# iostanin1/SCTL

Hardware: AMD Instinct MI355X
Metric: pair-interactions/s, Laplace-SL N x N direct sum (higher is better)
Workload: dtype f64; 1 GPU; Laplace3D single layer (Laplace3D-FxU), 2^20 x 2^20, fp64 [BASELINE headline / north_star target]; kernel=Laplace3D-FxU, n_trg=1048576, n_src=1048576, digits=-1

## Files before the change

include/sctl_amd/device/ukernels.hpp:

```cpp
#pragma once
#include <hip/hip_runtime.h>
#include <stdint.h>
#include <type_traits>

#include "fastmath.hpp"

namespace sctl_amd {

constexpr double kPi = 3.141592653589793238462643383279502884;

struct KerCtx { double v[4]; };

constexpr double kCubicC = 0x1.aaaaaa8000000p+0, kCubicK = 0x1.1c71c6e38e38ep+1;
constexpr double kCubic3C = 0x1.6666660000000p+0, kCubic3K = 0x1.7e4b170a3d700p-2, kCubic5C = 0x1.4924920000000p+0, kCubic5K = 0x1.2cee3c14e5e00p-3;
template <class R> struct RsqConst {
  R c38, c53, k209, c3, k3, c5, k5;
  __device__ __forceinline__ RsqConst() : c38(R(0.375)), c53(R(kCubicC)), k209(R(kCubicK)), c3(R(kCubic3C)), k3(R(kCubic3K)), c5(R(kCubic5C)), k5(R(kCubic5K)) {
    asm volatile("" : "+v"(c38), "+s"(c53), "+s"(k209), "+s"(c3), "+s"(k3), "+s"(c5), "+s"(k5));
  }
};

template <int MODE, bool MASKED> __device__ __forceinline__ double rsqrt_masked(double r2, const RsqConst<double>& K) {
  double y = __builtin_amdgcn_rsq(r2);
  if (MASKED) {
  int hi = __double2hiint(y);
  asm("" : "+v"(hi));
  hi = (hi == 0x7ff00000) ? 0 : hi;
  y = __hiloint2double(hi, __double2loint(y));
  }
  if (MODE >= 1) {
    const double a = r2 * y;
    const double e = __builtin_fma(-a, y, 1.0);
    const double ye = y * e;
    if (MODE == 1) y = __builtin_fma(ye, 0.5, y);
    else y = __builtin_fma(ye, __builtin_fma(e, K.c38, 0.5), y);
  }
  return y;
}
template <int MODE, bool MASKED> __device__ __forceinline__ float rsqrt_masked(float r2, const RsqConst<float>&) {
  float y = __builtin_amdgcn_rsqf(r2);
  if (MASKED) y = (__float_as_uint(y) == 0x7f800000u) ? 0.0f : y;
  if (MODE >= 1) {
    const float a = r2 * y;
    const float e = __builtin_fmaf(-a, y, 1.0f);
    y = __builtin_fmaf(y * e, 0.5f, y);
  }
  return y;
}

template <class R> struct DefaultConsts {
  static constexpr int LDS_DOUBLES = 0;
  static constexpr bool HAS_VARIANT = false;
  RsqConst<R> rsq;
  __device__ __forceinline__ explicit DefaultConsts(double*) {}
  __device__ __forceinline__ void begin_tile() const {}
  __device__ __forceinline__ bool tile_bad(const KerCtx&) const { return false; }
};
constexpr double helmholtz_dist_factor(int mode) { return mode == 1 ? 2.0 : mode == 2 ? 0x1.5555550000000p+1 : 1.0; }
template <class R> struct HelmholtzConsts;
template <> struct HelmholtzConsts<float> {
  static constexpr int LDS_DOUBLES = 0;
  static constexpr bool HAS_VARIANT = true;
  static constexpr int NUM_VARIANTS = 2;
  __device__ __forceinline__ int variant(const KerCtx& ctx) const { return ctx.v[1] == 0 ? 1 : 0; }
  RsqConst<float> rsq;
  float cinv = 1.0f;
  __device__ __forceinline__ explicit HelmholtzConsts(double*) {}
  __device__ __forceinline__ HelmholtzConsts(double*, int, const KerCtx&, int mode) : cinv((float)(1.0 / helmholtz_dist_factor(mode))) {}
  __device__ __forceinline__ void begin_tile() const {}
  __device__ __forceinline__ bool tile_bad(const KerCtx&) const { return false; }
};
template <> struct HelmholtzConsts<double> {
  static constexpr int LDS_DOUBLES = fastmath::kTableDoubles;
  static constexpr int LDS_DOUBLES_ALL_PAIRS = fastmath::kCexpTableDoubles > fastmath::kTableDoubles ? fastmath::kCexpTableDoubles : fastmath::kTableDoubles;
  static constexpr bool HAS_VARIANT = true;
  static constexpr int NUM_VARIANTS = 4;
  bool one_reduction;
  __device__ __forceinline__ int variant(const KerCtx& ctx) const { return (ctx.v[1] == 0 ? 1 : 0) + (one_reduction ? 2 : 0); }
  RsqConst<double> rsq;
  fastmath::TabCoeffsK tk;
  fastmath::CexpCoeffsK ck;
  const double* table;
  double cdist, cinv;
  __device__ __forceinline__ HelmholtzConsts(double* lds, int lds_doubles, const KerCtx& ctx) : HelmholtzConsts(lds, lds_doubles, ctx, 0) {}
  __device__ __forceinline__ HelmholtzConsts(double* lds, int lds_doubles, const KerCtx& ctx, int mode) : table(lds), cdist(helmholtz_dist_factor(mode)), cinv(1.0 / helmholtz_dist_factor(mode)) {
    one_reduction = lds_doubles >= fastmath::kCexpTableDoubles && fastmath::CexpCoeffsK::usable(ctx.v[0], -ctx.v[1]);
    {
      const fastmath::Coeffs full;
      if (one_reduction) fastmath::fill_cexp_tables(lds, (int)threadIdx.x, (int)blockDim.x, ctx.v[0], -ctx.v[1], full, fastmath::TabCoeffs());
      else fastmath::fill_tables(lds, (int)threadIdx.x, (int)blockDim.x, full);
    }
    __syncthreads();
    if (one_reduction) {
      ck.set_scaled(ctx.v[0], -ctx.v[1], fastmath::TabCoeffs(), cdist);
      ck.pin();
    } else {
      tk.set_scaled(ctx.v[0], -ctx.v[1], fastmath::TabCoeffs(), cdist);
      tk.pin();
    }
  }
  __device__ __forceinline__ HelmholtzConsts(double* lds, const KerCtx& ctx) : HelmholtzConsts(lds, LDS_DOUBLES, ctx) {}
  mutable unsigned rmax_hi = 0;
  __device__ __forceinline__ void begin_tile() const { rmax_hi = 0; }
  __device__ __forceinline__ void note_distance(double r) const {
    const unsigned h = (unsigned)__double2hiint(r);
    rmax_hi = (h > rmax_hi) ? h : rmax_hi;
  }
  __device__ __forceinline__ bool tile_bad(const KerCtx& ctx) const {
    const double rmax = __hiloint2double((int)(rmax_hi + 1u), 0);
    if (one_reduction) return !(ctx.v[0] * rmax <= fastmath::kCexpMaxPhase * cdist);
    return !(__builtin_fabs(ctx.v[0]) * rmax <= fastmath::kSincosTabMaxArg * cdist && __builtin_fabs(ctx.v[1]) * rmax <= fastmath::kExpTabMaxArg * cdist);
  }
};

template <class Ker, class R, int MODE, class = void, class = void> struct FinishOf {
  static __device__ __forceinline__ void apply(R (&)[Ker::K1]) {}
};
template <class Ker, class R, int MODE, class V> struct FinishOf<Ker, R, MODE, std::void_t<decltype(&Ker::template finish<R>)>, V> {
  static __device__ __forceinline__ void apply(R (&acc)[Ker::K1]) { Ker::template finish<R>(acc); }
};
template <class Ker, class R, int MODE> struct FinishOf<Ker, R, MODE, void, std::void_t<decltype(&Ker::template finish_mode<R, MODE>)>> {
  static __device__ __forceinline__ void apply(R (&acc)[Ker::K1]) { Ker::template finish_mode<R, MODE>(acc); }
};
template <class Ker, class R, int MODE> __device__ __forceinline__ void finish_acc(R (&acc)[Ker::K1]) { FinishOf<Ker, R, MODE>::apply(acc); }

template <class Ker, class R, int MODE, class = void> struct PackOf {
  static __device__ __forceinline__ void apply(R* rec, const R* x, const R* n, const R* f) { Ker::template pack<R>(rec, x, n, f); }
};
template <class Ker, class R, int MODE> struct PackOf<Ker, R, MODE, std::void_t<decltype(&Ker::template pack_mode<R, MODE>)>> {
  static __device__ __forceinline__ void apply(R* rec, const R* x, const R* n, const R* f) { Ker::template pack_mode<R, MODE>(rec, x, n, f); }
};
template <class Ker, class R, int MODE> __device__ __forceinline__ void pack_record(R* rec, const R* x, const R* n, const R* f) { PackOf<Ker, R, MODE>::apply(rec, x, n, f); }

template <class KC> __device__ __forceinline__ KC make_consts(double* lds, int lds_doubles, const KerCtx& ctx) {
  if constexpr (std::is_constructible<KC, double*, int, const KerCtx&>::value) return KC(lds, lds_doubles, ctx);
  else if constexpr (std::is_constructible<KC, double*, const KerCtx&>::value) return KC(lds, ctx);
  else return KC(lds);
}
template <class KC> __device__ __forceinline__ KC make_consts(double* lds, const KerCtx& ctx) { return make_consts<KC>(lds, KC::LDS_DOUBLES, ctx); }
template <class KC> __device__ __forceinline__ KC make_consts(double* lds, int lds_doubles, const KerCtx& ctx, int mode) {
  if constexpr (std::is_constructible<KC, double*, int, const KerCtx&, int>::value) return KC(lds, lds_doubles, ctx, mode);
  else return make_consts<KC>(lds, lds_doubles, ctx);
}
template <class KC> __device__ __forceinline__ KC make_consts(double* lds, const KerCtx& ctx, int mode) { return make_consts<KC>(lds, KC::LDS_DOUBLES, ctx, mode); }
template <class KC, class = void> struct AllPairsScratch { static constexpr int value = KC::LDS_DOUBLES; };
template <class KC> struct AllPairsScratch<KC, std::void_t<decltype(KC::LDS_DOUBLES_ALL_PAIRS)>> { static constexpr int value = KC::LDS_DOUBLES_ALL_PAIRS; };
template <class KC, class = void> struct NumVariants { static constexpr int value = KC::HAS_VARIANT ? 2 : 1; };
template <class KC> struct NumVariants<KC, std::void_t<decltype(KC::NUM_VARIANTS)>> { static constexpr int value = KC::NUM_VARIANTS; };

template <class R> __device__ __forceinline__ R fma_(R a, R b, R c);
template <> __device__ __forceinline__ double fma_<double>(double a, double b, double c) { return __builtin_fma(a, b, c); }
template <> __device__ __forceinline__ float fma_<float>(float a, float b, float c) { return __builtin_fmaf(a, b, c); }

template <class R> __device__ __forceinline__ R len2(const R (&d)[3]) { return fma_(d[2], d[2], fma_(d[1], d[1], d[0] * d[0])); }
template <class R> __device__ __forceinline__ R dot3(const R (&d)[3], const R* v) { return fma_(d[2], v[2], fma_(d[1], v[1], d[0] * v[0])); }

constexpr double kNewton2MeanErr = -1.725e-16;
constexpr double newton2_factor(int p) { return (p == 1 ? 2.0 : p == 3 ? 8.0 : 32.0) * (1.0 + p * kNewton2MeanErr); }
template <bool MASKED, class R> __device__ __forceinline__ R rsqrt_newton2(R r2, const RsqConst<R>& K) {
  const R y = rsqrt_masked<0, MASKED>(r2, K);
  const R a = r2 * y;
  return y * fma_(-a, y, R(3));
}

constexpr double cubic83_factor(int p) { return p == 1 ? 0x1.5555550000000p+1 : p == 3 ? 0x1.2f684af684bdep+4 : 0x1.0db20937d5dcdp+7; }
template <bool MASKED> __device__ __forceinline__ double rsqrt_cubic83(double r2, const RsqConst<double>& K) {
  const double y = rsqrt_masked<0, MASKED>(r2, K);
  const double z = __builtin_fma(r2, y * y, -K.c53);
  return y * __builtin_fma(z, z, K.k209);
}
template <bool MASKED> __device__ __forceinline__ float rsqrt_cubic83(float r2, const RsqConst<float>& K) { return rsqrt_masked<1, MASKED>(r2, K) * (float)cubic83_factor(1); }
template <int MODE, bool MASKED, class R> __device__ __forceinline__ R rsqrt_scaled(R r2, const RsqConst<R>& K) {
  if constexpr (MODE == 1) return rsqrt_newton2<MASKED>(r2, K);
  else if constexpr (MODE == 2) return rsqrt_cubic83<MASKED>(r2, K);
  else return rsqrt_masked<0, MASKED>(r2, K);
}
constexpr double rsqrt_scaled_factor(int mode, int p) { return mode == 1 ? newton2_factor(p) : mode == 2 ? cubic83_factor(p) : 1; }
constexpr double kCubic3A = 0x1.1111100000000p-1, kCubic5A = 0x1.d41d400000000p-3;
template <bool MASKED> __device__ __forceinline__ double rsqrt3_cubic(double r2, const RsqConst<double>& K) {
  const double y = rsqrt_masked<0, MASKED>(r2, K), s = y * y;
  const double z = __builtin_fma(r2, s, -K.c3);
  return (y * s) * __builtin_fma(z, z, K.k3);
}
template <bool MASKED> __device__ __forceinline__ double rsqrt5_cubic(double r2, const RsqConst<double>& K) {
  const double y = rsqrt_masked<0, MASKED>(r2, K), s = y * y;
  const double z = __builtin_fma(r2, s, -K.c5);
  return (y * (s * s)) * __builtin_fma(z, z, K.k5);
}
constexpr double rsqrt_pow_factor(int mode, int p) { return mode == 2 ? (p == 1 ? cubic83_factor(1) : p == 3 ? kCubic3A : kCubic5A) : rsqrt_scaled_factor(mode, p); }
template <int MODE, int P, bool MASKED, class R> __device__ __forceinline__ R rsqrt_pow_scaled(R r2, const RsqConst<R>& K) {
  static_assert(P == 3 || P == 5, "powers 3 and 5");
  if constexpr (MODE == 2 && std::is_same<R, double>::value) return P == 3 ? rsqrt3_cubic<MASKED>(r2, K) : rsqrt5_cubic<MASKED>(r2, K);
  else if constexpr (MODE == 2) {
    const R y = rsqrt_masked<1, MASKED>(r2, K), y2 = y * y;
    return (P == 3 ? y2 * y : y2 * y2 * y) * R(rsqrt_pow_factor(2, P));
  } else {
    const R y = rsqrt_scaled<MODE, MASKED>(r2, K), y2 = y * y;
    return P == 3 ? y2 * y : y2 * y2 * y;
  }
}

constexpr double rsqrt_scaled_c2(int mode) { return rsqrt_scaled_factor(mode, 1) == 1 ? 1.0 : mode == 1 ? 4.0 : cubic83_factor(1) * cubic83_factor(1); }


constexpr int nrec_multi(int nd, int k0, int m) { return (3 + nd + m * k0 + 1) / 2 * 2; }
template <int ND, int K0, class R, int M> __device__ __forceinline__ void pack_multi(R* rec, const R* x, const R* n, const R (&f)[M][K0]) {
  rec[0] = x[0]; rec[1] = x[1]; rec[2] = x[2];
#pragma unroll
  for (int k = 0; k < ND; k++) rec[3 + k] = n[k];
#pragma unroll
  for (int m = 0; m < M; m++)
#pragma unroll
    for (int k = 0; k < K0; k++) rec[3 + ND + m * K0 + k] = f[m][k];
}
#define SCTL_AMD_MULTI_RECORD                                                                                                          \
  template <int M> static constexpr int NREC_M = nrec_multi(ND, K0, M);                                                               \
  template <class R, int M> static __device__ __forceinline__ void pack_m(R* rec, const R* x, const R* n, const R (&f)[M][K0]) {      \
    pack_multi<ND, K0>(rec, x, n, f);                                                                                                 \
  }

struct Laplace3D_FxU {
  static constexpr int ID = 0, K0 = 1, K1 = 1, ND = 0, NREC = 4, FLOPS = 6;
  static constexpr const char* NAME = "Laplace3D-FxU";
  template <class R> using Consts = DefaultConsts<R>;
  static constexpr double scale() { return 1 / (4 * kPi); }
  static constexpr double acc_factor(int mode) { return rsqrt_scaled_factor(mode, 1); }
  template <class R> static __device__ __forceinline__ void pack(R* rec, const R* x, const R*, const R* f) {
    rec[0] = x[0]; rec[1] = x[1]; rec[2] = x[2]; rec[3] = f[0];
  }
  template <class R, int MODE, bool MASKED> static __device__ __forceinline__ void pair(R (&acc)[K1], const R (&d)[3], const R* rec, const KerCtx&, const Consts<R>& K) {
    const R rinv = rsqrt_scaled<MODE, MASKED>(len2(d), K.rsq);
    acc[0] = fma_(rec[3], rinv, acc[0]);
  }
  SCTL_AMD_MULTI_RECORD
  template <class R, int MODE, bool MASKED, int M> static __device__ __forceinline__ void pair_m(R (&acc)[M][K1], const R (&d)[3], const R* rec, const KerCtx&, const Consts<R>& K) {
    const R rinv = rsqrt_scaled<MODE, MASKED>(len2(d), K.rsq);
#pragma unroll
    for (int m = 0; m < M; m++) acc[m][0] = fma_(rec[3 + m], rinv, acc[m][0]);
  }
};

struct Laplace3D_DxU {
  static constexpr int ID = 1, K0 = 1, K1 = 1, ND = 3, NREC = 6, FLOPS = 14;
  static constexpr const char* NAME = "Laplace3D-DxU";
  template <class R> using Consts = DefaultConsts<R>;
  static constexpr double scale() { return 1 / (4 * kPi); }
  static constexpr double acc_factor(int mode) { return rsqrt_pow_factor(mode, 3); }
  template <class R> static __device__ __forceinline__ void pack(R* rec, const R* x, const R* n, const R* f) {
    rec[0] = x[0]; rec[1] = x[1]; rec[2] = x[2]; rec[3] = n[0] * f[0]; rec[4] = n[1] * f[0]; rec[5] = n[2] * f[0];
  }
  template <class R, int MODE, bool MASKED> static __device__ __forceinline__ void pair(R (&acc)[K1], const R (&d)[3], const R* rec, const KerCtx&, const Consts<R>& K) {
    acc[0] = fma_(dot3(d, rec + 3), rsqrt_pow_scaled<MODE, 3, MASKED>(len2(d), K.rsq), acc[0]);
  }
  SCTL_AMD_MULTI_RECORD
  template <class R, int MODE, bool MASKED, int M> static __device__ __forceinline__ void pair_m(R (&acc)[M][K1], const R (&d)[3], const R* rec, const KerCtx&, const Consts<R>& K) {
    const R t = dot3(d, rec + 3) * rsqrt_pow_scaled<MODE, 3, MASKED>(len2(d), K.rsq);
#pragma unroll
    for (int m = 0; m < M; m++) acc[m][0] = fma_(rec[6 + m], t, acc[m][0]);
  }
};

struct Laplace3D_FxdU {
  static constexpr int ID = 2, K0 = 1, K1 = 3, ND = 0, NREC = 4, FLOPS = 11;
  static constexpr const char* NAME = "Laplace3D-FxdU";
  template <class R> using Consts = DefaultConsts<R>;
  static constexpr double scale() { return -1 / (4 * kPi); }
  static constexpr double acc_factor(int mode) { return rsqrt_pow_factor(mode, 3); }
  template <class R> static __device__ __forceinline__ void pack(R* rec, const R* x, const R*, const R* f) {
    rec[0] = x[0]; rec[1] = x[1]; rec[2] = x[2]; rec[3] = f[0];
  }
  template <class R, int MODE, bool MASKED> static __device__ __forceinline__ void pair(R (&acc)[K1], const R (&d)[3], const R* rec, const KerCtx&, const Consts<R>& K) {
    const R t = rsqrt_pow_scaled<MODE, 3, MASKED>(len2(d), K.rsq) * rec[3];
    for (int j = 0; j < 3; j++) acc[j] = fma_(t, d[j], acc[j]);
  }
  SCTL_AMD_MULTI_RECORD
  template <class R, int MODE, bool MASKED, int M> static __device__ __forceinline__ void pair_m(R (&acc)[M][K1], const R (&d)[3], const R* rec, const KerCtx&, const Consts<R>& K) {
    const R t = rsqrt_pow_scaled<MODE, 3, MASKED>(len2(d), K.rsq);
    const R td[3] = {t * d[0], t * d[1], t * d[2]};
#pragma unroll
    for (int m = 0; m < M; m++)
#pragma unroll
      for (int j = 0; j < 3; j++) acc[m][j] = fma_(rec[3 + m], td[j], acc[m][j]);
  }
};

struct Stokes3D_FxU {
  static constexpr int ID = 3, K0 = 3, K1 = 3, ND = 0, NREC = 10, FLOPS = 23;
  static constexpr const char* NAME = "Stokes3D-FxU";
  template <class R> using Consts = DefaultConsts<R>;
  static constexpr double scale() { return 1 / (8 * kPi); }
  static constexpr double acc_factor(int mode) { return rsqrt_scaled_factor(mode, 3); }
  template <class R, int MODE> static __device__ __forceinline__ void pack_mode(R* rec, const R* x, const R*, const R* f) {
    const R c2 = R(rsqrt_scaled_c2(MODE));
    rec[0] = x[0]; rec[1] = x[1]; rec[2] = x[2]; rec[3] = f[0]; rec[4] = f[1]; rec[5] = f[2]; rec[6] = c2 * f[0]; rec[7] = c2 * f[1]; rec[8] = c2 * f[2]; rec[9] = 0;
  }
  template <class R> static __device__ __forceinline__ void pack(R* rec, const R* x, const R* n, const R* f) { pack_mode<R, 0>(rec, x, n, f); }
  template <class R, int MODE, bool MASKED> static __device__ __forceinline__ void pair(R (&acc)[K1], const R (&d)[3], const R* rec, const KerCtx&, const Consts<R>& K) {
    const R y = rsqrt_scaled<MODE, MASKED>(len2(d), K.rsq);
    const R t = dot3(d, rec + 3) * (y * y);
    for (int j = 0; j < 3; j++) acc[j] = fma_(y, fma_(t, d[j], rec[6 + j]), acc[j]);
  }
  SCTL_AMD_MULTI_RECORD
  template <class R, int MODE, bool MASKED, int M> static __device__ __forceinline__ void pair_m(R (&acc)[M][K1], const R (&d)[3], const R* rec, const KerCtx&, const Consts<R>& K) {
    const R y = rsqrt_scaled<MODE, MASKED>(len2(d), K.rsq);
    const R y3 = (y * y) * y;
    const R yc = (rsqrt_scaled_c2(MODE) == 1.0) ? y : y * R(rsqrt_scaled_c2(MODE));
    const R e[3] = {y3 * d[0], y3 * d[1], y3 * d[2]};
#pragma unroll
    for (int m = 0; m < M; m++) {
      const R* f = rec + 3 + 3 * m;
      const R rf = dot3(d, f);
#pragma unroll
      for (int j = 0; j < 3; j++) acc[m][j] = fma_(e[j], rf, fma_(yc, f[j], acc[m][j]));
    }
  }
};

struct Stokes3D_DxU {
  static constexpr int ID = 4, K0 = 3, K1 = 3, ND = 3, NREC = 10, FLOPS = 26;
  static constexpr const char* NAME = "Stokes3D-DxU";
  template <class R> using Consts = DefaultConsts<R>;
  static constexpr double scale() { return 3 / (4 * kPi); }
  static constexpr double acc_factor(int mode) { return rsqrt_pow_factor(mode, 5); }
  template <class R> static __device__ __forceinline__ void pack(R* rec, const R* x, const R* n, const R* f) {
    for (int k = 0; k < 3; k++) { rec[k] = x[k]; rec[3 + k] = n[k]; rec[6 + k] = f[k]; }
    rec[9] = 0;
  }
  template <class R, int MODE, bool MASKED> static __device__ __forceinline__ void pair(R (&acc)[K1], const R (&d)[3], const R* rec, const KerCtx&, const Consts<R>& K) {
// ... 284 lines not shown
```

sctl_amd/csrc/centered_kernel.hpp:

```cpp
#pragma once
#include <sctl_amd/device/eval_kernel.hpp>

namespace sctl_amd {

constexpr double kNearFactor2 = 4.0;

template <class R> __device__ __forceinline__ R wave_min(R v) {
  for (int o = 32; o > 0; o >>= 1) { const R w = __shfl_xor(v, o); v = (w < v) ? w : v; }
  return v;
}
template <class R> __device__ __forceinline__ R wave_max(R v) {
  for (int o = 32; o > 0; o >>= 1) { const R w = __shfl_xor(v, o); v = (w > v) ? w : v; }
  return v;
}

__device__ __forceinline__ double uniform_(double v) {
  return __hiloint2double(__builtin_amdgcn_readfirstlane(__double2hiint(v)), __builtin_amdgcn_readfirstlane(__double2loint(v)));
}
__device__ __forceinline__ float uniform_(float v) { return __int_as_float(__builtin_amdgcn_readfirstlane(__float_as_int(v))); }
__device__ __forceinline__ double sqrt_(double v) { return __builtin_sqrt(v); }
__device__ __forceinline__ float sqrt_(float v) { return __builtin_sqrtf(v); }

template <class R> struct Rec4;
template <> struct Rec4<double> {
  typedef double V __attribute__((ext_vector_type(2)));
  static constexpr int NW = 2;
  static __device__ __forceinline__ void put(V* p, double a, double b, double c, double d) { p[0] = V{a, b}; p[1] = V{c, d}; }
  static __device__ __forceinline__ void get(const V* p, double (&o)[4]) { const V u = p[0], w = p[1]; o[0] = u[0]; o[1] = u[1]; o[2] = w[0]; o[3] = w[1]; }
};
template <> struct Rec4<float> {
  typedef float V __attribute__((ext_vector_type(4)));
  static constexpr int NW = 1;
  static __device__ __forceinline__ void put(V* p, float a, float b, float c, float d) { p[0] = V{a, b, c, d}; }
  static __device__ __forceinline__ void get(const V* p, float (&o)[4]) { const V u = p[0]; o[0] = u[0]; o[1] = u[1]; o[2] = u[2]; o[3] = u[3]; }
};

constexpr int kWaveBlock = 64;
constexpr int kWaveTile = 64;
#if defined(SCTL_AMD_EXPERIMENTS) && defined(SCTL_AMD_EXP_NEARCAP)
constexpr int kNearCap = SCTL_AMD_EXP_NEARCAP;
static_assert(kNearCap >= 64, "a tile of 64 sources must fit the list of pending near sources");
#else
constexpr int kNearCap = 128;
#endif

typedef float f32x2 __attribute__((ext_vector_type(2)));
template <int MODE, int P = 1> __device__ __forceinline__ f32x2 rsqrt_pair(f32x2 r2) {
  f32x2 y = {__builtin_amdgcn_rsqf(r2[0]), __builtin_amdgcn_rsqf(r2[1])};
  if (MODE >= 1) {
    const f32x2 a = r2 * y;
    y = y * (f32x2{3.0f, 3.0f} - a * y);
    if (MODE == 2) {
      const float k = (float)__builtin_pow(rsqrt_pow_factor(2, P), 1.0 / P) / 2;
      y = y * f32x2{k, k};
    }
  }
  return y;
}
__device__ __forceinline__ f32x2 pk_add_hi(f32x2 t, f32x2 zA) {
  f32x2 r;
  asm("v_pk_add_f32 %0, %1, %2 op_sel:[0,1] op_sel_hi:[1,1]" : "=v"(r) : "v"(t), "v"(zA));
  return r;
}
__device__ __forceinline__ f32x2 pk_fma_lo_hi(f32x2 m, f32x2 g) {
  f32x2 r;
  asm("v_pk_fma_f32 %0, %1, %2, %2 op_sel:[0,0,1] op_sel_hi:[1,0,1]" : "=v"(r) : "v"(m), "v"(g));
  return r;
}

template <class R, int T> struct FarTargets {
  R m2x[T][3], tt[T];
  __device__ __forceinline__ void set(int j, const R (&p)[3], R t2) {
    tt[j] = t2;
#pragma unroll
    for (int k = 0; k < 3; k++) m2x[j][k] = R(-2) * p[k];
  }
};
template <> struct FarTargets<float, 2> {
  f32x2 mp[3], tp;
  __device__ __forceinline__ void set(int j, const float (&p)[3], float t2) {
    tp[j] = t2;
#pragma unroll
    for (int k = 0; k < 3; k++) mp[k][j] = -2.0f * p[k];
  }
};

template <class R> struct CenteredFxU {
  using Ker = Laplace3D_FxU;
  static constexpr bool DUP = std::is_same<R, float>::value;
  static constexpr int XW = DUP ? 2 : 1, NF = 1, NEAR_CAP = 128;
  template <class RR> static constexpr int targets_per_lane() { return sizeof(RR) == 8 ? 4 : 2; }
  struct Extra { R f, f2; };
  template <int MODE> static __device__ __forceinline__ void put_extra(R* base, int q, const R (&)[3], const R*, const R* f) {
    if (DUP) { base[2 * q] = f[0]; base[2 * q + 1] = f[0]; }
    else base[q] = f[0];
  }
  static __device__ __forceinline__ void put_null(R* base, int q) {
    if (DUP) { base[2 * q] = R(0); base[2 * q + 1] = R(0); }
    else base[q] = R(0);
  }
  static __device__ __forceinline__ Extra load_extra(const R* base, int s) { return DUP ? Extra{base[2 * s], base[2 * s + 1]} : Extra{base[s], R(0)}; }
  static __device__ __forceinline__ void store_extra(R* base, int q, const Extra& e) {
    if (DUP) { base[2 * q] = e.f; base[2 * q + 1] = e.f2; }
    else base[q] = e.f;
  }
  template <int MODE> static __device__ __forceinline__ void far_pair(R& acc, const R (&m2x)[3], R tt, const R (&b)[4], const Extra& e, const RsqConst<R>& K) {
    const R r2 = fma_(m2x[0], b[0], fma_(m2x[1], b[1], fma_(m2x[2], b[2], tt + b[3])));
    acc = fma_(e.f, rsqrt_scaled<MODE, false>(r2, K), acc);
  }
  template <int MODE, int T, class KC> static __device__ __forceinline__ void far_pairs(R (&acc)[T][NF], const FarTargets<R, T>& tg, const R (&b)[4], const Extra& e,
                                                                                          const KC& K) {
    if constexpr (std::is_same<R, float>::value && T == 2) {
      f32x2 r2 = pk_add_hi(tg.tp, f32x2{b[2], b[3]});
      r2 = tg.mp[2] * f32x2{b[2], b[2]} + r2;
      r2 = tg.mp[1] * f32x2{b[1], b[1]} + r2;
      r2 = tg.mp[0] * f32x2{b[0], b[0]} + r2;
      const f32x2 a = f32x2{acc[0][0], acc[1][0]} + f32x2{e.f, e.f2} * rsqrt_pair<MODE>(r2);
      acc[0][0] = a[0]; acc[1][0] = a[1];
    } else {
#pragma unroll
      for (int j = 0; j < T; j++) far_pair<MODE>(acc[j][0], tg.m2x[j], tg.tt[j], b, e, K.rsq);
    }
  }
};
template <class R> struct CenteredDxU {
  using Ker = Laplace3D_DxU;
  static constexpr int XW = 4, NF = 1, NEAR_CAP = 128;
  template <class RR> static constexpr int targets_per_lane() { return sizeof(RR) == 8 ? 4 : 2; }
  struct Extra { R g[4]; };
  template <int MODE> static __device__ __forceinline__ void put_extra(R* base, int q, const R (&p)[3], const R* n, const R* f) {
    const R nf[3] = {n[0] * f[0], n[1] * f[0], n[2] * f[0]};
    Rec4<R>::put((typename Rec4<R>::V*)base + q * Rec4<R>::NW, R(-0.5) * nf[0], R(-0.5) * nf[1], R(-0.5) * nf[2], -(p[0] * nf[0] + p[1] * nf[1] + p[2] * nf[2]));
  }
  static __device__ __forceinline__ void put_null(R* base, int q) { Rec4<R>::put((typename Rec4<R>::V*)base + q * Rec4<R>::NW, R(0), R(0), R(0), R(0)); }
  static __device__ __forceinline__ Extra load_extra(const R* base, int s) {
    Extra e;
    Rec4<R>::get((const typename Rec4<R>::V*)base + s * Rec4<R>::NW, e.g);
    return e;
  }
  static __device__ __forceinline__ void store_extra(R* base, int q, const Extra& e) {
    Rec4<R>::put((typename Rec4<R>::V*)base + q * Rec4<R>::NW, e.g[0], e.g[1], e.g[2], e.g[3]);
  }
  template <int MODE> static __device__ __forceinline__ void far_pair(R& acc, const R (&m2x)[3], R tt, const R (&b)[4], const Extra& e, const RsqConst<R>& K) {
    const R r2 = fma_(m2x[0], b[0], fma_(m2x[1], b[1], fma_(m2x[2], b[2], tt + b[3])));
    const R y3 = rsqrt_pow_scaled<MODE, 3, false>(r2, K);
    const R dn = fma_(m2x[0], e.g[0], fma_(m2x[1], e.g[1], fma_(m2x[2], e.g[2], e.g[3])));
    acc = fma_(dn, y3, acc);
  }
  template <int MODE, int T, class KC> static __device__ __forceinline__ void far_pairs(R (&acc)[T][NF], const FarTargets<R, T>& tg, const R (&b)[4], const Extra& e,
                                                                                          const KC& K) {
    if constexpr (std::is_same<R, float>::value && T == 2) {
      const f32x2 mx = tg.mp[0], my = tg.mp[1], mz = tg.mp[2];
      f32x2 r2 = pk_add_hi(tg.tp, f32x2{b[2], b[3]});
      r2 = mz * f32x2{b[2], b[2]} + r2;
      r2 = my * f32x2{b[1], b[1]} + r2;
      r2 = mx * f32x2{b[0], b[0]} + r2;
      const f32x2 y = rsqrt_pair<MODE, 3>(r2);
      f32x2 dn = pk_fma_lo_hi(mz, f32x2{e.g[2], e.g[3]});
      dn = my * f32x2{e.g[1], e.g[1]} + dn;
      dn = mx * f32x2{e.g[0], e.g[0]} + dn;
      const f32x2 a = f32x2{acc[0][0], acc[1][0]} + dn * (y * y * y);
      acc[0][0] = a[0]; acc[1][0] = a[1];
    } else {
#pragma unroll
      for (int j = 0; j < T; j++) far_pair<MODE>(acc[j][0], tg.m2x[j], tg.tt[j], b, e, K.rsq);
    }
  }
};

template <class R, int XW> struct ExtraWords {
  static_assert(XW % 4 == 0, "whole Rec4 groups");
  struct Extra { R g[XW]; };
  static __device__ __forceinline__ Extra load_extra(const R* base, int s) {
    Extra e;
#pragma unroll
    for (int w = 0; w < XW / 4; w++) {
      R v[4];
      Rec4<R>::get((const typename Rec4<R>::V*)base + (s * (XW / 4) + w) * Rec4<R>::NW, v);
      e.g[4 * w] = v[0]; e.g[4 * w + 1] = v[1]; e.g[4 * w + 2] = v[2]; e.g[4 * w + 3] = v[3];
    }
    return e;
  }
  static __device__ __forceinline__ void store_extra(R* base, int q, const Extra& e) {
#pragma unroll
    for (int w = 0; w < XW / 4; w++)
      Rec4<R>::put((typename Rec4<R>::V*)base + (q * (XW / 4) + w) * Rec4<R>::NW, e.g[4 * w], e.g[4 * w + 1], e.g[4 * w + 2], e.g[4 * w + 3]);
  }
  static __device__ __forceinline__ void put_null(R* base, int q) {
    Extra e;
#pragma unroll
    for (int k = 0; k < XW; k++) e.g[k] = R(0);
    store_extra(base, q, e);
  }
};
template <class R> struct CenteredFxdU : ExtraWords<R, 4> {
  using Ker = Laplace3D_FxdU;
  using Extra = typename ExtraWords<R, 4>::Extra;
  static constexpr int XW = 4, NF = 4, NEAR_CAP = 128;
  template <class RR> static constexpr int targets_per_lane() { return 3; }
  template <int MODE> static __device__ __forceinline__ void put_extra(R* base, int q, const R (&p)[3], const R*, const R* f) {
    Extra e{{f[0], f[0] * p[0], f[0] * p[1], f[0] * p[2]}};
    ExtraWords<R, 4>::store_extra(base, q, e);
  }
  template <int MODE, int T, class KC> static __device__ __forceinline__ void far_pairs(R (&acc)[T][NF], const FarTargets<R, T>& tg, const R (&b)[4], const Extra& e,
                                                                                          const KC& K) {
#pragma unroll
    for (int j = 0; j < T; j++) {
      const R r2 = fma_(tg.m2x[j][0], b[0], fma_(tg.m2x[j][1], b[1], fma_(tg.m2x[j][2], b[2], tg.tt[j] + b[3])));
      const R y3 = rsqrt_pow_scaled<MODE, 3, false>(r2, K.rsq);
#pragma unroll
      for (int k = 0; k < 4; k++) acc[j][k] = fma_(y3, e.g[k], acc[j][k]);
    }
  }
  template <int MODE> static __device__ __forceinline__ void finish(R (&out)[3], const R (&far)[NF], const R (&near)[3], const R (&m2x)[3]) {
#pragma unroll
    for (int k = 0; k < 3; k++) out[k] = near[k] + fma_(R(-0.5) * m2x[k], far[0], -far[1 + k]);
  }
};
template <class R, class KER> struct CenteredStokeslet : ExtraWords<R, 8> {
  using Ker = KER;
  using Extra = typename ExtraWords<R, 8>::Extra;
  static constexpr int XW = 8, NF = 4, NEAR_CAP = 64;
  static_assert(KER::K0 == 3 || KER::K0 == 4, "three force components, optionally a source/sink strength");
  static_assert(KER::K1 == 3 || KER::K1 == 4, "velocity, optionally the pressure");
  template <class RR> static constexpr int targets_per_lane() { return 4; }
  template <int MODE> static __device__ __forceinline__ void put_extra(R* base, int q, const R (&p)[3], const R*, const R* f) {
    const R c2 = R(rsqrt_scaled_c2(MODE));
    R g3 = -(p[0] * f[0] + p[1] * f[1] + p[2] * f[2]);
    if constexpr (KER::K0 == 4) g3 += f[3];
    Extra e{{R(-0.5) * f[0], R(-0.5) * f[1], R(-0.5) * f[2], g3, c2 * f[0], c2 * f[1], c2 * f[2], R(0)}};
    ExtraWords<R, 8>::store_extra(base, q, e);
  }
  template <int MODE, int T, class KC> static __device__ __forceinline__ void far_pairs(R (&acc)[T][NF], const FarTargets<R, T>& tg, const R (&b)[4], const Extra& e,
                                                                                          const KC& K) {
#pragma unroll
    for (int j = 0; j < T; j++) {
      const R r2 = fma_(tg.m2x[j][0], b[0], fma_(tg.m2x[j][1], b[1], fma_(tg.m2x[j][2], b[2], tg.tt[j] + b[3])));
      const R y = rsqrt_scaled<MODE, false>(r2, K.rsq);
      const R t = fma_(tg.m2x[j][0], e.g[0], fma_(tg.m2x[j][1], e.g[1], fma_(tg.m2x[j][2], e.g[2], e.g[3]))) * (y * y);
      acc[j][3] = fma_(t, y, acc[j][3]);
#pragma unroll
      for (int k = 0; k < 3; k++) acc[j][k] = fma_(y, fma_(-t, b[k], e.g[4 + k]), acc[j][k]);
    }
  }
  template <int MODE> static __device__ __forceinline__ void finish(R (&out)[KER::K1], const R (&far)[NF], const R (&near)[KER::K1], const R (&m2x)[3]) {
#pragma unroll
    for (int k = 0; k < 3; k++) out[k] = near[k] + fma_(R(-0.5) * m2x[k], far[3], far[k]);
    if constexpr (KER::K1 == 4) out[3] = near[3] + far[3];
  }
};

__device__ __forceinline__ void centered_tile_and_split(unsigned& tile_idx, unsigned& split_idx) {
  tile_idx = blockIdx.x; split_idx = blockIdx.y;
  if ((gridDim.y & 7u) == 0) {
    const unsigned b = blockIdx.y * gridDim.x + blockIdx.x, xcd = b & 7u, j = b >> 3, per = gridDim.y >> 3;
    tile_idx = j % gridDim.x;
    split_idx = xcd * per + j / gridDim.x;
  }
}
template <class CP, class R, int MODE, int T, int UNR = 4>
__global__ void __launch_bounds__(kWaveBlock) centered_kernel(const EvalArgs<R> a) {
  using V = typename Rec4<R>::V;
  constexpr int NW = Rec4<R>::NW;
  using Ker = typename CP::Ker;
  constexpr int ND = Ker::ND, K0 = Ker::K0, K1 = Ker::K1, NF = CP::NF;
  constexpr bool SCALAR = (K1 == 1 && NF == 1);
  constexpr int kNearCap = CP::NEAR_CAP < sctl_amd::kNearCap ? CP::NEAR_CAP : sctl_amd::kNearCap;
  constexpr int NEARW = (Ker::NREC + 3) / 4;
  constexpr int XV = (CP::XW * (int)sizeof(R) + 15) / 16;
  __shared__ V farB[(kWaveTile + UNR) * NW];
  __shared__ V farXv[(kWaveTile + UNR) * (XV > 0 ? XV : 1)];
  __shared__ V nearA[(kNearCap + 2) * NW * NEARW];
  R* const farX = (R*)farXv;

  const int lane = threadIdx.x;
  unsigned tile_idx, split_idx;
  centered_tile_and_split(tile_idx, split_idx);
  const int64_t tbase = (int64_t)tile_idx * (kWaveBlock * T);
  const typename Ker::template Consts<R> K(nullptr);

  R xt[T][3];
  R c[3];
  {
    R lo[3] = {max_finite<R>(), max_finite<R>(), max_finite<R>()}, hi[3] = {-lo[0], -lo[0], -lo[0]};
#pragma unroll
    for (int j = 0; j < T; j++) {
      int64_t t = tbase + j * kWaveBlock + lane;
      if (t >= a.Nt) t = a.Nt - 1;
#pragma unroll
      for (int k = 0; k < 3; k++) {
        xt[j][k] = a.xt[t * 3 + k];
        lo[k] = (xt[j][k] < lo[k]) ? xt[j][k] : lo[k];
        hi[k] = (xt[j][k] > hi[k]) ? xt[j][k] : hi[k];
      }
    }
#pragma unroll
    for (int k = 0; k < 3; k++) c[k] = uniform_(R(0.5) * wave_min(lo[k]) + R(0.5) * wave_max(hi[k]));
  }
  FarTargets<R, T> tg;
  R rt2 = 0;
#pragma unroll
  for (int j = 0; j < T; j++) {
    const R p[3] = {xt[j][0] - c[0], xt[j][1] - c[1], xt[j][2] - c[2]};
    const R t2 = len2(p);
    rt2 = (t2 > rt2) ? t2 : rt2;
    tg.set(j, p, t2);
  }
  rt2 = uniform_(wave_max(rt2));
  const R near_r2 = R(a.ctx.v[0]) * rt2;

  R acc[T][K1];
  R facc[T][SCALAR ? 1 : NF];
#pragma unroll
  for (int j = 0; j < T; j++) {
#pragma unroll
    for (int k = 0; k < K1; k++) acc[j][k] = 0;
#pragma unroll
    for (int k = 0; k < (SCALAR ? 1 : NF); k++) facc[j][k] = 0;
  }

  const int64_t s_begin = (int64_t)split_idx * a.chunk;
  const int64_t s_end = (s_begin + a.chunk < a.Ns) ? s_begin + a.chunk : a.Ns;
  const int64_t len = (s_end > s_begin) ? s_end - s_begin : 0;
  const int ntile = (int)((len + kWaveTile - 1) / kWaveTile);

  R x[3] = {0, 0, 0}, nrm[3] = {0, 0, 0}, f[K0];
#pragma unroll
  for (int k = 0; k < K0; k++) f[k] = 0;
  auto load_source = [&](int it) {
    const int64_t s = s_begin + (int64_t)it * kWaveTile + lane;
    if (s < s_end) {
#pragma unroll
      for (int k = 0; k < 3; k++) x[k] = a.xs[s * 3 + k];
#pragma unroll
      for (int k = 0; k < ND; k++) nrm[k] = a.xn[s * ND + k];
#pragma unroll
      for (int k = 0; k < K0; k++) f[k] = a.f[s * K0 + k];
    }
  };
  if (ntile > 0) load_source(0);

  const R far_off = R(1.0e3) * (R(1) + sqrt_(rt2));
  auto put_near = [&](int q, const R (&xq)[3], const R (&nq)[3], const R (&fq)[K0]) {
    R rec[4 * NEARW] = {};
    pack_record<Ker, R, MODE>(rec, xq, nq, fq);
#pragma unroll
    for (int g = 0; g < NEARW; g++) Rec4<R>::put(nearA + (q * NEARW + g) * NW, rec[4 * g], rec[4 * g + 1], rec[4 * g + 2], rec[4 * g + 3]);
  };
  int nn = 0;
  auto flush_near = [&]() {
    if (nn & 1) {
      if (lane == 0) {
        const R xq[3] = {c[0] + far_off, c[1], c[2]}, nq[3] = {0, 0, 0}, fq[K0] = {};
        put_near(nn, xq, nq, fq);
      }
      __syncthreads();
    }
    R xo[T][3];
#pragma unroll
    for (int j = 0; j < T; j++) {
      int64_t t = tbase + j * kWaveBlock + lane;
      if (t >= a.Nt) t = a.Nt - 1;
#pragma unroll
      for (int k = 0; k < 3; k++) xo[j][k] = a.xt[t * 3 + k];
    }
    for (int s = 0; s < nn; s += 2) {
#pragma unroll
      for (int u = 0; u < 2; u++) {
        R q[4 * NEARW];
#pragma unroll
        for (int g = 0; g < NEARW; g++) {
          R w[4];
          Rec4<R>::get(nearA + ((s + u) * NEARW + g) * NW, w);
          q[4 * g] = w[0]; q[4 * g + 1] = w[1]; q[4 * g + 2] = w[2]; q[4 * g + 3] = w[3];
        }
#pragma unroll
        for (int j = 0; j < T; j++) {
          const R d[3] = {xo[j][0] - q[0], xo[j][1] - q[1], xo[j][2] - q[2]};
          Ker::template pair<R, MODE, true>(acc[j], d, q, a.ctx, K);
#if !(defined(SCTL_AMD_EXPERIMENTS) && defined(SCTL_AMD_EXP_NO_NEAR_FENCE))
          __builtin_amdgcn_sched_barrier(0);
#endif
        }
      }
    }
    nn = 0;
  };

  auto stage_tile = [&](int it, int carry) -> int {
    const int ns = (it == ntile - 1) ? (int)(len - (int64_t)it * kWaveTile) : kWaveTile;
    const bool valid = lane < ns;
    const R p[3] = {x[0] - c[0], x[1] - c[1], x[2] - c[2]};
    const R ss = len2(p);
    const bool is_far = valid && (ss > near_r2);
    const bool is_near = valid && !is_far;
    const unsigned long long bf = __ballot(is_far), bn = __ballot(is_near);
    const unsigned long long below = (lane == 0) ? 0ull : (~0ull >> (64 - lane));
    const int nfar = __popcll(bf), nnear = __popcll(bn);
    __syncthreads();
    if (nn + nnear > kNearCap) {
      flush_near();
      __syncthreads();
    }
    if (is_far) {
      const int q = carry + __popcll(bf & below);
      Rec4<R>::put(farB + q * NW, p[0], p[1], p[2], ss);
      CP::template put_extra<MODE>(farX, q, p, nrm, f);
    } else if (is_near) {
      put_near(nn + __popcll(bn & below), x, nrm, f);
    }
    nn += nnear;
    return nfar;
  };
  auto run_far = [&](int m) {
    R tacc[T][NF];
#pragma unroll
    for (int j = 0; j < T; j++)
#pragma unroll
      for (int k = 0; k < NF; k++) tacc[j][k] = 0;
    for (int s = 0; s < m; s += UNR) {
#pragma unroll
      for (int u = 0; u < UNR; u++) {
        R b[4];
        Rec4<R>::get(farB + (s + u) * NW, b);
        const typename CP::Extra e = CP::load_extra(farX, s + u);
        CP::template far_pairs<MODE, T>(tacc, tg, b, e, K);
      }
    }
#pragma unroll
    for (int j = 0; j < T; j++) {
      if constexpr (SCALAR) acc[j][0] += tacc[j][0];
      else {
#pragma unroll
        for (int k = 0; k < NF; k++) facc[j][k] += tacc[j][k];
      }
    }
  };
  auto put_null_far = [&](int q) { Rec4<R>::put(farB + q * NW, far_off, R(0), R(0), far_off * far_off); CP::put_null(farX, q); };

  if constexpr (sizeof(R) == 8) {
    int carry = 0;
    for (int it = 0; it < ntile; it++) {
      const int n = carry + stage_tile(it, carry), m = n & ~(UNR - 1);
      if (it + 1 < ntile) load_source(it + 1);
      __syncthreads();
      run_far(m);
      carry = n - m;
      if (m > 0 && lane < carry) {
        R b[4];
        Rec4<R>::get(farB + (m + lane) * NW, b);
        const typename CP::Extra e = CP::load_extra(farX, m + lane);
        Rec4<R>::put(farB + lane * NW, b[0], b[1], b[2], b[3]);
        CP::store_extra(farX, lane, e);
      }
    }
    __syncthreads();
    if (carry > 0) {
      if (lane < UNR - carry) put_null_far(carry + lane);
      __syncthreads();
      run_far(UNR);
    }
  } else {
    for (int it = 0; it < ntile; it++) {
      const int nfar = stage_tile(it, 0), padded = (nfar + UNR - 1) & ~(UNR - 1);
      if (lane < UNR - 1 && nfar + lane < padded) put_null_far(nfar + lane);
      if (it + 1 < ntile) load_source(it + 1);
      __syncthreads();
      run_far(padded);
    }
  }
  __syncthreads();
  flush_near();

#pragma unroll
  for (int j = 0; j < T; j++) {
    const int64_t t = tbase + j * kWaveBlock + lane;
    if constexpr (SCALAR) {
      if (t < a.Nt) {
        if (gridDim.y == 1) a.v_trg[t] += acc[j][0] * a.scale;
        else a.partial[(int64_t)split_idx * a.Nt + t] = acc[j][0];
      }
    } else {
      R out[K1];
      CP::template finish<MODE>(out, facc[j], acc[j], tg.m2x[j]);
      finish_acc<Ker, R, MODE>(out);
      if (t < a.Nt) {
#pragma unroll
        for (int k = 0; k < K1; k++) {
          if (gridDim.y == 1) a.v_trg[t * K1 + k] += out[k] * a.scale;
          else a.partial[((int64_t)split_idx * a.Nt + t) * K1 + k] = out[k];
        }
      }
    }
  }
}

template <class R> __global__ void __launch_bounds__(kBlock) bbox_partial_kernel(const R* x, int64_t n, double* part) {
  __shared__ double red[4 * 6];
  double lo[3] = {1.7976931348623157e308, 1.7976931348623157e308, 1.7976931348623157e308}, hi[3] = {-lo[0], -lo[0], -lo[0]};
  for (int64_t i = (int64_t)blockIdx.x * kBlock + threadIdx.x; i < n; i += (int64_t)gridDim.x * kBlock) {
#pragma unroll
    for (int k = 0; k < 3; k++) {
      const double v = (double)x[i * 3 + k];
      lo[k] = (v < lo[k]) ? v : lo[k];
      hi[k] = (v > hi[k]) ? v : hi[k];
    }
  }
#pragma unroll
  for (int k = 0; k < 3; k++) { lo[k] = wave_min(lo[k]); hi[k] = wave_max(hi[k]); }
  const int lane = threadIdx.x & 63, wave = threadIdx.x >> 6;
  if (lane == 0) {
#pragma unroll
    for (int k = 0; k < 3; k++) { red[wave * 6 + k] = lo[k]; red[wave * 6 + 3 + k] = hi[k]; }
  }
  __syncthreads();
  if (threadIdx.x < 6) {
    const int k = threadIdx.x;
    double v = red[k];
    for (int w = 1; w < 4; w++) v = (k < 3) ? ((red[w * 6 + k] < v) ? red[w * 6 + k] : v) : ((red[w * 6 + k] > v) ? red[w * 6 + k] : v);
    part[blockIdx.x * 6 + k] = v;
  }
}

__device__ __forceinline__ uint64_t spread21(uint64_t v) {
  v &= 0x1fffffull;
  v = (v | (v << 32)) & 0x1f00000000ffffull;
  v = (v | (v << 16)) & 0x1f0000ff0000ffull;
  v = (v | (v << 8)) & 0x100f00f00f00f00full;
  v = (v | (v << 4)) & 0x10c30c30c30c30c3ull;
  v = (v | (v << 2)) & 0x1249249249249249ull;
  return v;
}

template <class R> __global__ void __launch_bounds__(kBlock) morton_keys_kernel(const R* x, int64_t n, const double* part, int nblk, uint64_t* keys, uint32_t* idx) {
  __shared__ double box[6];
  if (threadIdx.x < 6) {
    const int k = threadIdx.x;
    double v = part[k];
    for (int b = 1; b < nblk; b++) v = (k < 3) ? ((part[b * 6 + k] < v) ? part[b * 6 + k] : v) : ((part[b * 6 + k] > v) ? part[b * 6 + k] : v);
    box[k] = v;
  }
  __syncthreads();
  const int64_t i = (int64_t)blockIdx.x * kBlock + threadIdx.x;
  if (i >= n) return;
  uint64_t key = 0;
#pragma unroll
  for (int k = 0; k < 3; k++) {
    const double w = box[3 + k] - box[k];
    const double q = (w > 0) ? ((double)x[i * 3 + k] - box[k]) / w * 2097151.0 : 0.0;
    const uint64_t qi = (q > 0) ? (uint64_t)((q < 2097151.0) ? q : 2097151.0) : 0ull;
    key |= spread21(qi) << k;
  }
  keys[i] = key;
  idx[i] = (uint32_t)i;
}

template <class R> __global__ void __launch_bounds__(kBlock) gather_points_kernel(const R* x, const uint32_t* perm, int64_t n, R* out) {
  const int64_t i = (int64_t)blockIdx.x * kBlock + threadIdx.x;
  if (i >= n) return;
  const int64_t s = perm[i];
#pragma unroll
  for (int k = 0; k < 3; k++) out[i * 3 + k] = x[s * 3 + k];
}

template <class R> __global__ void __launch_bounds__(kBlock) scatter_add_kernel(const R* sorted, const uint32_t* perm, int64_t n, int k1, R* v_trg) {
  const int64_t i = (int64_t)blockIdx.x * kBlock + threadIdx.x;
  if (i >= n) return;
  const int64_t t = perm[i];
  for (int k = 0; k < k1; k++) v_trg[t * k1 + k] += sorted[i * k1 + k];
}

}
```

Measured before the change: 2823 billion pair-interactions/s.

## Fold source density into scaled far records for the fp64 single-layer kernel

For the fp64 Laplace single-layer centered kernel, each far source's record is scaled by k=1/f^2, so that rsqrt(k*r2) equals |f|/r. This removes the per-pair multiply by the density. Sources are split by sign into two stacks that grow from either end of the LDS tile, and the sign is applied as a compile-time negation, so the rsqrt split form can fuse its final multiply into the accumulate FMA. Sources with zero density are dropped. Sources whose scaling would fall outside a safe exponent range are sent to the near path. The cost is a more complex staging and carry scheme, an extra division per source, and two loops per tile, one for each sign.

```diff
diff --git a/include/sctl_amd/device/ukernels.hpp b/include/sctl_amd/device/ukernels.hpp
--- a/include/sctl_amd/device/ukernels.hpp
+++ b/include/sctl_amd/device/ukernels.hpp
@@ -157,23 +157,37 @@
 
 constexpr double kNewton2MeanErr = -1.725e-16;
 constexpr double newton2_factor(int p) { return (p == 1 ? 2.0 : p == 3 ? 8.0 : 32.0) * (1.0 + p * kNewton2MeanErr); }
-template <bool MASKED, class R> __device__ __forceinline__ R rsqrt_newton2(R r2, const RsqConst<R>& K) {
+template <class R> struct RsqSplit { R y, p; };
+template <bool MASKED, class R> __device__ __forceinline__ RsqSplit<R> rsqrt_newton2_split(R r2, const RsqConst<R>& K) {
   const R y = rsqrt_masked<0, MASKED>(r2, K);
   const R a = r2 * y;
-  return y * fma_(-a, y, R(3));
+  return {y, fma_(-a, y, R(3))};
+}
+template <bool MASKED, class R> __device__ __forceinline__ R rsqrt_newton2(R r2, const RsqConst<R>& K) {
+  const RsqSplit<R> s = rsqrt_newton2_split<MASKED>(r2, K);
+  return s.y * s.p;
 }
 
 constexpr double cubic83_factor(int p) { return p == 1 ? 0x1.5555550000000p+1 : p == 3 ? 0x1.2f684af684bdep+4 : 0x1.0db20937d5dcdp+7; }
-template <bool MASKED> __device__ __forceinline__ double rsqrt_cubic83(double r2, const RsqConst<double>& K) {
+template <bool MASKED> __device__ __forceinline__ RsqSplit<double> rsqrt_cubic83_split(double r2, const RsqConst<double>& K) {
   const double y = rsqrt_masked<0, MASKED>(r2, K);
   const double z = __builtin_fma(r2, y * y, -K.c53);
-  return y * __builtin_fma(z, z, K.k209);
+  return {y, __builtin_fma(z, z, K.k209)};
+}
+template <bool MASKED> __device__ __forceinline__ double rsqrt_cubic83(double r2, const RsqConst<double>& K) {
+  const RsqSplit<double> s = rsqrt_cubic83_split<MASKED>(r2, K);
+  return s.y * s.p;
 }
 template <bool MASKED> __device__ __forceinline__ float rsqrt_cubic83(float r2, const RsqConst<float>& K) { return rsqrt_masked<1, MASKED>(r2, K) * (float)cubic83_factor(1); }
 template <int MODE, bool MASKED, class R> __device__ __forceinline__ R rsqrt_scaled(R r2, const RsqConst<R>& K) {
   if constexpr (MODE == 1) return rsqrt_newton2<MASKED>(r2, K);
   else if constexpr (MODE == 2) return rsqrt_cubic83<MASKED>(r2, K);
   else return rsqrt_masked<0, MASKED>(r2, K);
+}
+template <int MODE, bool MASKED> __device__ __forceinline__ RsqSplit<double> rsqrt_scaled_split(double r2, const RsqConst<double>& K) {
+  if constexpr (MODE == 1) return rsqrt_newton2_split<MASKED>(r2, K);
+  else if constexpr (MODE == 2) return rsqrt_cubic83_split<MASKED>(r2, K);
+  else return {rsqrt_masked<0, MASKED>(r2, K), 1.0};
 }
 constexpr double rsqrt_scaled_factor(int mode, int p) { return mode == 1 ? newton2_factor(p) : mode == 2 ? cubic83_factor(p) : 1; }
 constexpr double kCubic3A = 0x1.1111100000000p-1, kCubic5A = 0x1.d41d400000000p-3;
diff --git a/sctl_amd/csrc/centered_kernel.hpp b/sctl_amd/csrc/centered_kernel.hpp
--- a/sctl_amd/csrc/centered_kernel.hpp
+++ b/sctl_amd/csrc/centered_kernel.hpp
@@ -104,13 +104,34 @@
     if (DUP) { base[2 * q] = e.f; base[2 * q + 1] = e.f2; }
     else base[q] = e.f;
   }
+  static constexpr bool FOLD = !DUP;
+  static __device__ __forceinline__ int fold_class(R f, R ss, R& k) {
+    if (f == R(0)) return 0;
+    k = R(1) / (f * f);
+    const R kss = k * ss;
+    if (!(kss >= R(0x1p-600) && kss <= R(0x1p600) && ss >= R(0x1p-300) && ss <= R(0x1p300))) return 2;
+    return f > R(0) ? 1 : -1;
+  }
+  static __device__ __forceinline__ void put_folded(typename Rec4<R>::V* rec, R* base, int q, const R (&p)[3], R ss, R k) {
+    Rec4<R>::put(rec + q * Rec4<R>::NW, k * p[0], k * p[1], k * p[2], k * ss);
+    base[q] = k;
+  }
   template <int MODE> static __device__ __forceinline__ void far_pair(R& acc, const R (&m2x)[3], R tt, const R (&b)[4], const Extra& e, const RsqConst<R>& K) {
     const R r2 = fma_(m2x[0], b[0], fma_(m2x[1], b[1], fma_(m2x[2], b[2], tt + b[3])));
     acc = fma_(e.f, rsqrt_scaled<MODE, false>(r2, K), acc);
   }
-  template <int MODE, int T, class KC> static __device__ __forceinline__ void far_pairs(R (&acc)[T][NF], const FarTargets<R, T>& tg, const R (&b)[4], const Extra& e,
-                                                                                          const KC& K) {
-    if constexpr (std::is_same<R, float>::value && T == 2) {
+  template <int MODE, bool NEG> static __device__ __forceinline__ void far_pair_folded(R& acc, const R (&m2x)[3], R tt, const R (&b)[4], const Extra& e,
+                                                                                       const RsqConst<R>& K) {
+    const R r2 = fma_(m2x[0], b[0], fma_(m2x[1], b[1], fma_(m2x[2], b[2], fma_(tt, e.f, b[3]))));
+    const RsqSplit<R> s = rsqrt_scaled_split<MODE, false>(r2, K);
+    acc = fma_(NEG ? -s.y : s.y, s.p, acc);
+  }
+  template <int MODE, int T, bool NEG = false, class KC> static __device__ __forceinline__ void far_pairs(R (&acc)[T][NF], const FarTargets<R, T>& tg, const R (&b)[4],
+                                                                                                          const Extra& e, const KC& K) {
+    if constexpr (FOLD) {
+#pragma unroll
+      for (int j = 0; j < T; j++) far_pair_folded<MODE, NEG>(acc[j][0], tg.m2x[j], tg.tt[j], b, e, K.rsq);
+    } else if constexpr (std::is_same<R, float>::value && T == 2) {
       f32x2 r2 = pk_add_hi(tg.tp, f32x2{b[2], b[3]});
       r2 = tg.mp[2] * f32x2{b[2], b[2]} + r2;
       r2 = tg.mp[1] * f32x2{b[1], b[1]} + r2;
@@ -258,6 +279,9 @@
     split_idx = xcd * per + j / gridDim.x;
   }
 }
+template <class CP, class = void> struct FoldsDensity : std::false_type {};
+template <class CP> struct FoldsDensity<CP, std::void_t<decltype(CP::FOLD)>> : std::integral_constant<bool, CP::FOLD> {};
+
 template <class CP, class R, int MODE, int T, int UNR = 4>
 __global__ void __launch_bounds__(kWaveBlock) centered_kernel(const EvalArgs<R> a) {
   using V = typename Rec4<R>::V;
@@ -268,8 +292,10 @@
   constexpr int kNearCap = CP::NEAR_CAP < sctl_amd::kNearCap ? CP::NEAR_CAP : sctl_amd::kNearCap;
   constexpr int NEARW = (Ker::NREC + 3) / 4;
   constexpr int XV = (CP::XW * (int)sizeof(R) + 15) / 16;
-  __shared__ V farB[(kWaveTile + UNR) * NW];
-  __shared__ V farXv[(kWaveTile + UNR) * (XV > 0 ? XV : 1)];
+  constexpr bool FOLD = FoldsDensity<CP>::value;
+  constexpr int FAR_CAP = FOLD ? kWaveTile + 2 * (UNR - 1) : kWaveTile + UNR;
+  __shared__ V farB[FAR_CAP * NW];
+  __shared__ V farXv[FAR_CAP * (XV > 0 ? XV : 1)];
   __shared__ V nearA[(kNearCap + 2) * NW * NEARW];
   R* const farX = (R*)farXv;
 
@@ -438,7 +464,96 @@
   };
   auto put_null_far = [&](int q) { Rec4<R>::put(farB + q * NW, far_off, R(0), R(0), far_off * far_off); CP::put_null(farX, q); };
 
-  if constexpr (sizeof(R) == 8) {
+  if constexpr (FOLD) {
+    static_assert(SCALAR && NF == 1, "the fold is the single layer's");
+    auto stage_tile_folded = [&](int it, int cpos, int cneg, int& npos, int& nneg) {
+      const int ns = (it == ntile - 1) ? (int)(len - (int64_t)it * kWaveTile) : kWaveTile;
+      const bool valid = lane < ns;
+      const R p[3] = {x[0] - c[0], x[1] - c[1], x[2] - c[2]};
+      const R ss = len2(p);
+      const bool far = valid && (ss > near_r2);
+      R k = 0;
+      const int cls = far ? CP::fold_class(f[0], ss, k) : 2;
+      const bool is_pos = far && cls == 1, is_neg = far && cls == -1, is_near = valid && cls == 2;
+      const unsigned long long bp = __ballot(is_pos), bq = __ballot(is_neg), bn = __ballot(is_near);
+      const unsigned long long below = (lane == 0) ? 0ull : (~0ull >> (64 - lane));
+      const int nnear = __popcll(bn);
+      __syncthreads();
+      if (nn + nnear > kNearCap) {
+        flush_near();
+        __syncthreads();
+      }
+      if (is_pos) CP::put_folded(farB, farX, cpos + __popcll(bp & below), p, ss, k);
+      else if (is_neg) CP::put_folded(farB, farX, FAR_CAP - 1 - (cneg + __popcll(bq & below)), p, ss, k);
+      else if (is_near) put_near(nn + __popcll(bn & below), x, nrm, f);
+      nn += nnear;
+      npos = __popcll(bp);
+      nneg = __popcll(bq);
+    };
+    auto far_folded = [&](R (&tacc)[T][NF], int i, auto neg) {
+      constexpr bool NEG = decltype(neg)::value;
+      const int q = NEG ? FAR_CAP - 1 - i : i;
+      R b[4];
+      Rec4<R>::get(farB + q * NW, b);
+      const typename CP::Extra e = CP::load_extra(farX, q);
+      CP::template far_pairs<MODE, T, NEG>(tacc, tg, b, e, K);
+    };
+    auto run_far_folded = [&](int mp, int mn) {
+      R tacc[T][NF];
+#pragma unroll
+      for (int j = 0; j < T; j++) tacc[j][0] = 0;
+      const std::integral_constant<bool, false> pos;
+      const std::integral_constant<bool, true> neg;
+      const int mb = mp < mn ? mp : mn;
+      int s = 0;
+      for (; s < mb; s += UNR) {
+#pragma unroll
+        for (int u = 0; u < UNR; u++) far_folded(tacc, s + u, pos);
+#pragma unroll
+        for (int u = 0; u < UNR; u++) far_folded(tacc, s + u, neg);
+      }
+      for (; s < mp; s += UNR) {
+#pragma unroll
+        for (int u = 0; u < UNR; u++) far_folded(tacc, s + u, pos);
+      }
+      for (; s < mn; s += UNR) {
+#pragma unroll
+        for (int u = 0; u < UNR; u++) far_folded(tacc, s + u, neg);
+      }
+#pragma unroll
+      for (int j = 0; j < T; j++) acc[j][0] += tacc[j][0];
+    };
+    int cpos = 0, cneg = 0;
+    for (int it = 0; it < ntile; it++) {
+      int npos, nneg;
+      stage_tile_folded(it, cpos, cneg, npos, nneg);
+      const int np = cpos + npos, nq = cneg + nneg, mp = np & ~(UNR - 1), mq = nq & ~(UNR - 1);
+      if (it + 1 < ntile) load_source(it + 1);
+      __syncthreads();
+      run_far_folded(mp, mq);
+      cpos = np - mp;
+      cneg = nq - mq;
+      const bool mv_pos = mp > 0 && lane < cpos, mv_neg = mq > 0 && lane >= 32 && lane < 32 + cneg;
+      if (mv_pos || mv_neg) {
+        const int from = mv_pos ? mp + lane : FAR_CAP - 1 - (mq + lane - 32), to = mv_pos ? lane : FAR_CAP - 1 - (lane - 32);
+        R b[4];
+        Rec4<R>::get(farB + from * NW, b);
+        const typename CP::Extra e = CP::load_extra(farX, from);
+        Rec4<R>::put(farB + to * NW, b[0], b[1], b[2], b[3]);
+        CP::store_extra(farX, to, e);
+      }
+    }
+    __syncthreads();
+    if (cpos + cneg > 0) {
+      R tacc[T][NF];
+#pragma unroll
+      for (int j = 0; j < T; j++) tacc[j][0] = 0;
+      for (int i = 0; i < cpos; i++) far_folded(tacc, i, std::integral_constant<bool, false>());
+      for (int i = 0; i < cneg; i++) far_folded(tacc, i, std::integral_constant<bool, true>());
+#pragma unroll
+      for (int j = 0; j < T; j++) acc[j][0] += tacc[j][0];
+    }
+  } else if constexpr (sizeof(R) == 8) {
     int carry = 0;
     for (int it = 0; it < ntile; it++) {
       const int n = carry + stage_tile(it, carry), m = n & ~(UNR - 1);
```

Measured after the change: 3002 billion pair-interactions/s (median of 6 runs). 6.3% higher.
